# RiccZamboni/mepol

Hardware: AMD Instinct MI355X
Metric: MEPOL epoch wall-clock (C3: N=200000, d=29, k=30; rollout excluded) (lower is better)
Workload: dtype f64; 1 GPU; C3 Ant-shaped MEPOL epoch (k-NN + off-policy loop + final H); particles=200000, num_traj=400, traj_len=500, d=29, k=30, policy=29->[400, 300]->8 f64, parallelism=dp1

## Files before the change

### mepol_amd/csrc/wgrad.hip

```cpp
#include "mfma_f64.hpp"

#include <algorithm>

namespace mepol {
namespace wgrad {

using mfma::d4;
using mfma::frag_col;
using mfma::frag_row;
constexpr int FO = 4, FI = 5;
constexpr int kOcc = 2;
constexpr int BO = 16 * FO, BI = 16 * FI;
constexpr int NL = FO + FI;
constexpr int NS = 2;
constexpr bool kPin = true;
constexpr int kMaxSlices = 128;
constexpr int kSliceRowsMin = 256;

inline int slices_for(int64_t n, int O, int I) {
  const int64_t ntile = (int64_t)((O + BO - 1) / BO) * ((I + BI - 1) / BI);
  int64_t s = std::max<int64_t>(8, 1024 * kOcc / ntile);
  s = std::min<int64_t>(s, std::max<int64_t>(8, n / kSliceRowsMin));
  return (int)std::min<int64_t>(kMaxSlices, s & ~7);
}

inline size_t ws_bytes(int64_t n, int O, int I) {
  return (size_t)slices_for(n, O, I) * O * I * sizeof(double);
}

__global__ __launch_bounds__(64) __attribute__((amdgpu_waves_per_eu(kOcc))) void wgrad_kernel(
    const double* __restrict__ dy, int64_t n, int O, const double* __restrict__ x, int I,
    int nob, int nib, int S, int64_t slice_rows, double* __restrict__ part) {
  const int ntile = nob * nib;
  const int64_t b = blockIdx.x;
  const int64_t j = b >> 3;
  const int64_t s = (j / ntile) * 8 + (b & 7);
  const int tile = (int)(j % ntile);
  if (s >= S) return;
  const int ob = tile / nib, ib = tile % nib;
  const int l = threadIdx.x, fr = l & 15, g = l >> 4;
  const int64_t r_begin = s * slice_rows;
  const int64_t r_end = min(n, r_begin + slice_rows);
  if (r_begin >= r_end) {
    for (int t = 0; t < FO; ++t)
      for (int q = 0; q < 4; ++q) {
        const int o = ob * BO + 16 * t + frag_row(l, q);
        for (int u = 0; u < FI; ++u) {
          const int i = ib * BI + 16 * u + frag_col(l);
          if (o < O && i < I) part[((int64_t)s * O + o) * I + i] = 0.0;
        }
      }
    return;
  }
  int oc[FO], ic[FI];
#pragma unroll
  for (int t = 0; t < FO; ++t) oc[t] = min(ob * BO + 16 * t + fr, O - 1);
#pragma unroll
  for (int u = 0; u < FI; ++u) ic[u] = min(ib * BI + 16 * u + fr, I - 1);

  d4 acc[FO][FI];
#pragma unroll
  for (int t = 0; t < FO; ++t)
#pragma unroll
    for (int u = 0; u < FI; ++u) acc[t][u] = d4{0.0, 0.0, 0.0, 0.0};

  double R[NS][NL];
  auto load = [&](double (&D)[NL], int64_t ks) __attribute__((always_inline)) {
    const int64_t r = min(r_begin + 4 * ks + g, r_end - 1);
    const double* yr = dy + r * O;
    const double* xr = x + r * I;
#pragma unroll
    for (int t = 0; t < FO; ++t) D[t] = yr[oc[t]];
#pragma unroll
    for (int u = 0; u < FI; ++u) D[FO + u] = xr[ic[u]];
  };
  auto mma = [&](const double (&D)[NL]) __attribute__((always_inline)) {
#pragma unroll
    for (int t = 0; t < FO; ++t)
#pragma unroll
      for (int u = 0; u < FI; ++u)
        acc[t][u] = __builtin_amdgcn_mfma_f64_16x16x4f64(D[t], D[FO + u], acc[t][u], 0, 0, 0);
  };
  const int64_t rows = r_end - r_begin;
  const int64_t nfull = rows / 4;
  const int64_t nks = (rows + 3) / 4;
  mfma::ring_k_loop<NS, kPin>(
      nfull, nks, [&](int p, int64_t ks) __attribute__((always_inline)) { load(R[p], ks); },
      [&](int p, int64_t ks) __attribute__((always_inline)) {
        const bool ok = r_begin + 4 * ks + g < r_end;
#pragma unroll
        for (int v = 0; v < NL; ++v) R[p][v] = ok ? R[p][v] : 0.0;
      },
      [&](int p) __attribute__((always_inline)) { mma(R[p]); });
#pragma unroll
  for (int t = 0; t < FO; ++t)
#pragma unroll
    for (int q = 0; q < 4; ++q) {
      const int o = ob * BO + 16 * t + frag_row(l, q);
#pragma unroll
      for (int u = 0; u < FI; ++u) {
        const int i = ib * BI + 16 * u + frag_col(l);
        if (o < O && i < I) part[((int64_t)s * O + o) * I + i] = acc[t][u][q];
      }
    }
}

__global__ __launch_bounds__(256) void wgrad_reduce_kernel(const double* __restrict__ part, int S,
                                                          int64_t elems, double* __restrict__ out) {
  const int64_t e = (int64_t)blockIdx.x * 256 + threadIdx.x;
  if (e >= elems) return;
  double v = 0.0;
  for (int s = 0; s < S; s += 8) {
    double p[8];
#pragma unroll
    for (int u = 0; u < 8; ++u) p[u] = part[(int64_t)(s + u) * elems + e];
#pragma unroll
    for (int u = 0; u < 8; ++u) v += p[u];
  }
  out[e] = v;
}

}
}

extern "C" int mepol_weight_grad_workspace_size(int64_t n, int out_features, int in_features,
                                                size_t* bytes) {
  if (!bytes || n < 0 || out_features <= 0 || in_features <= 0) return mepol::kErrBadArg;
  *bytes = mepol::wgrad::ws_bytes(n, out_features, in_features);
  return 0;
}

extern "C" int mepol_weight_grad(const double* dy, int64_t n, int out_features, const double* x,
                                 int in_features, double* dW, void* workspace,
                                 size_t workspace_bytes, void* stream) {
  using namespace mepol::wgrad;
  const int O = out_features, I = in_features;
  if (n <= 0 || O <= 0 || I <= 0 || !dy || !x || !dW || !workspace) {
    mepol::set_error("mepol_weight_grad: bad arguments");
    return mepol::kErrBadArg;
  }
  const int S = slices_for(n, O, I);
  const size_t need = ws_bytes(n, O, I);
  if (workspace_bytes < need) {
    mepol::set_error("mepol_weight_grad: workspace %zu < %zu", workspace_bytes, need);
    return mepol::kErrWorkspace;
  }
  hipStream_t st = (hipStream_t)stream;
  const int nob = (O + BO - 1) / BO, nib = (I + BI - 1) / BI;
  const int64_t slice_rows = ((n + S - 1) / S + 3) / 4 * 4;
  const unsigned blocks = (unsigned)((int64_t)S * nob * nib);
  double* part = (double*)workspace;
  hipLaunchKernelGGL(wgrad_kernel, dim3(blocks), dim3(64), 0, st, dy, n, O, x, I, nob, nib, S,
                     slice_rows, part);
  MEPOL_CHECK_LAUNCH();
  const int64_t elems = (int64_t)O * I;
  hipLaunchKernelGGL(wgrad_reduce_kernel, dim3((unsigned)((elems + 255) / 256)), dim3(256), 0, st,
                     part, S, elems, dW);
  MEPOL_CHECK_LAUNCH();
  return 0;
}
```

Before: 0.1023 s/epoch.

## Split wgrad into full and short output tiles with XCD-aware slice scheduling

The weight-gradient kernel now handles the partial last output-row block separately, with a templated tile width (FOV) so short tiles issue fewer MFMAs and use a deeper pipeline. A host-side plan picks different split-K slice counts for full and short tiles and spreads blocks across the 8 XCDs with per-XCD capacity accounting. The reduce kernel is updated for the two partial layouts and non-multiple-of-8 slice counts. This aims to cut wasted MFMA work on padded rows and balance load across XCDs, at the cost of more complex scheduling logic and a kernel-wide branch.

```diff
diff --git a/mepol_amd/csrc/wgrad.hip b/mepol_amd/csrc/wgrad.hip
--- a/mepol_amd/csrc/wgrad.hip
+++ b/mepol_amd/csrc/wgrad.hip
@@ -11,75 +11,133 @@
 constexpr int FO = 4, FI = 5;
 constexpr int kOcc = 2;
 constexpr int BO = 16 * FO, BI = 16 * FI;
-constexpr int NL = FO + FI;
 constexpr int NS = 2;
+constexpr int kShortStages = 3;
 constexpr bool kPin = true;
 constexpr int kMaxSlices = 128;
 constexpr int kSliceRowsMin = 256;
 
-inline int slices_for(int64_t n, int O, int I) {
-  const int64_t ntile = (int64_t)((O + BO - 1) / BO) * ((I + BI - 1) / BI);
-  int64_t s = std::max<int64_t>(8, 1024 * kOcc / ntile);
-  s = std::min<int64_t>(s, std::max<int64_t>(8, n / kSliceRowsMin));
-  return (int)std::min<int64_t>(kMaxSlices, s & ~7);
+struct XcdMap {
+  int fend[8], send[8], fbase[8], sbase[8];
+};
+struct Plan {
+  int nob, nib, fol;
+  int Sf, Ss;
+  int64_t rows_f, rows_s;
+  int grid8;
+  XcdMap m;
+};
+constexpr int kXcdWaves = 1024 / 8 * kOcc;
+
+inline int64_t slice_rows_of(int64_t n, int S) { return ((n + S - 1) / S + 3) / 4 * 4; }
+
+inline Plan plan_for(int64_t n, int O, int I) {
+  Plan p{};
+  p.nob = (O + BO - 1) / BO;
+  p.nib = (I + BI - 1) / BI;
+  p.fol = (O - BO * (p.nob - 1) + 15) / 16;
+  const int nfo = p.nob - 1;
+  const int64_t lim = std::max<int64_t>(8, n / kSliceRowsMin);
+  const int64_t slots = 8 * kXcdWaves;
+  int64_t want_s;
+  if (nfo > 0) {
+    const int64_t sf = 4 * slots / ((int64_t)p.nib * (4 * nfo + p.fol));
+    p.Sf = (int)std::min<int64_t>({(int64_t)kMaxSlices, lim, std::max<int64_t>(8, sf)});
+    if ((int64_t)((p.Sf + 7) / 8) * nfo * p.nib > kXcdWaves) p.Sf = std::max(8, p.Sf & ~7);
+    want_s = ((int64_t)p.Sf * p.fol + 3) / 4;
+  } else {
+    want_s = slots / p.nib;
+  }
+  want_s = std::min<int64_t>({(int64_t)kMaxSlices, lim, std::max<int64_t>(8, want_s)});
+  const int tf = nfo * p.nib, ts = p.nib;
+  int nf[8], cap[8], ns[8];
+  int64_t capsum = 0;
+  for (int x = 0; x < 8; ++x) {
+    nf[x] = p.Sf / 8 + (x < p.Sf % 8 ? 1 : 0);
+    cap[x] = std::max(0, (kXcdWaves - nf[x] * tf) / ts);
+    capsum += cap[x];
+    ns[x] = 0;
+  }
+  if (capsum < 8)
+    for (int x = 0; x < 8; ++x) cap[x] = kMaxSlices;
+  else
+    want_s = std::min(want_s, capsum);
+  p.Ss = (int)want_s;
+  for (int left = p.Ss, x = 7; left > 0; x = (x + 7) % 8)
+    if (ns[x] < cap[x]) {
+      ++ns[x];
+      --left;
+    }
+  int fb = 0, sb = 0;
+  for (int x = 0; x < 8; ++x) {
+    p.m.fend[x] = nf[x] * tf;
+    p.m.send[x] = p.m.fend[x] + ns[x] * ts;
+    p.m.fbase[x] = fb;
+    p.m.sbase[x] = sb;
+    fb += nf[x];
+    sb += ns[x];
+    p.grid8 = std::max(p.grid8, p.m.send[x]);
+  }
+  p.rows_f = p.Sf ? slice_rows_of(n, p.Sf) : 0;
+  p.rows_s = slice_rows_of(n, p.Ss);
+  return p;
 }
 
 inline size_t ws_bytes(int64_t n, int O, int I) {
-  return (size_t)slices_for(n, O, I) * O * I * sizeof(double);
-}
-
-__global__ __launch_bounds__(64) __attribute__((amdgpu_waves_per_eu(kOcc))) void wgrad_kernel(
-    const double* __restrict__ dy, int64_t n, int O, const double* __restrict__ x, int I,
-    int nob, int nib, int S, int64_t slice_rows, double* __restrict__ part) {
-  const int ntile = nob * nib;
-  const int64_t b = blockIdx.x;
-  const int64_t j = b >> 3;
-  const int64_t s = (j / ntile) * 8 + (b & 7);
-  const int tile = (int)(j % ntile);
-  if (s >= S) return;
-  const int ob = tile / nib, ib = tile % nib;
+  const Plan p = plan_for(n, O, I);
+  const int64_t of = (int64_t)BO * (p.nob - 1);
+  return (size_t)(p.Sf * of + p.Ss * (O - of)) * I * sizeof(double);
+}
+
+template <int FOV>
+__device__ __forceinline__ void wgrad_tile(const double* __restrict__ dy, int64_t n, int O,
+                                           const double* __restrict__ x, int I, int o0, int g0,
+                                           int og, int ib, int64_t s, int64_t slice_rows,
+                                           double* __restrict__ part) {
+  constexpr int NLV = FOV + FI;
+  constexpr int NS = FOV < FO ? kShortStages : wgrad::NS;
   const int l = threadIdx.x, fr = l & 15, g = l >> 4;
   const int64_t r_begin = s * slice_rows;
   const int64_t r_end = min(n, r_begin + slice_rows);
   if (r_begin >= r_end) {
-    for (int t = 0; t < FO; ++t)
+    for (int t = 0; t < FOV; ++t)
       for (int q = 0; q < 4; ++q) {
-        const int o = ob * BO + 16 * t + frag_row(l, q);
+        const int o = o0 + 16 * t + frag_row(l, q);
         for (int u = 0; u < FI; ++u) {
           const int i = ib * BI + 16 * u + frag_col(l);
-          if (o < O && i < I) part[((int64_t)s * O + o) * I + i] = 0.0;
+          if (o < O && i < I) part[((int64_t)s * og + o - g0) * I + i] = 0.0;
         }
       }
     return;
   }
-  int oc[FO], ic[FI];
-#pragma unroll
-  for (int t = 0; t < FO; ++t) oc[t] = min(ob * BO + 16 * t + fr, O - 1);
+  int oc[FOV], ic[FI];
+#pragma unroll
+  for (int t = 0; t < FOV; ++t) oc[t] = min(o0 + 16 * t + fr, O - 1);
 #pragma unroll
   for (int u = 0; u < FI; ++u) ic[u] = min(ib * BI + 16 * u + fr, I - 1);
 
-  d4 acc[FO][FI];
-#pragma unroll
-  for (int t = 0; t < FO; ++t)
+  d4 acc[FOV][FI];
+#pragma unroll
+  for (int t = 0; t < FOV; ++t)
 #pragma unroll
     for (int u = 0; u < FI; ++u) acc[t][u] = d4{0.0, 0.0, 0.0, 0.0};
 
-  double R[NS][NL];
-  auto load = [&](double (&D)[NL], int64_t ks) __attribute__((always_inline)) {
+  double R[NS][NLV];
+  auto load = [&](double (&D)[NLV], int64_t ks) __attribute__((always_inline)) {
     const int64_t r = min(r_begin + 4 * ks + g, r_end - 1);
     const double* yr = dy + r * O;
     const double* xr = x + r * I;
 #pragma unroll
-    for (int t = 0; t < FO; ++t) D[t] = yr[oc[t]];
-#pragma unroll
-    for (int u = 0; u < FI; ++u) D[FO + u] = xr[ic[u]];
+    for (int t = 0; t < FOV; ++t) D[t] = yr[oc[t]];
+#pragma unroll
+    for (int u = 0; u < FI; ++u) D[FOV + u] = xr[ic[u]];
   };
-  auto mma = [&](const double (&D)[NL]) __attribute__((always_inline)) {
-#pragma unroll
-    for (int t = 0; t < FO; ++t)
+  auto mma = [&](const double (&D)[NLV]) __attribute__((always_inline)) {
+#pragma unroll
+    for (int t = 0; t < FOV; ++t)
 #pragma unroll
       for (int u = 0; u < FI; ++u)
-        acc[t][u] = __builtin_amdgcn_mfma_f64_16x16x4f64(D[t], D[FO + u], acc[t][u], 0, 0, 0);
+        acc[t][u] = __builtin_amdgcn_mfma_f64_16x16x4f64(D[t], D[FOV + u], acc[t][u], 0, 0, 0);
   };
   const int64_t rows = r_end - r_begin;
   const int64_t nfull = rows / 4;
@@ -89,33 +147,70 @@
       [&](int p, int64_t ks) __attribute__((always_inline)) {
         const bool ok = r_begin + 4 * ks + g < r_end;
 #pragma unroll
-        for (int v = 0; v < NL; ++v) R[p][v] = ok ? R[p][v] : 0.0;
+        for (int v = 0; v < NLV; ++v) R[p][v] = ok ? R[p][v] : 0.0;
       },
       [&](int p) __attribute__((always_inline)) { mma(R[p]); });
 #pragma unroll
-  for (int t = 0; t < FO; ++t)
+  for (int t = 0; t < FOV; ++t)
 #pragma unroll
     for (int q = 0; q < 4; ++q) {
-      const int o = ob * BO + 16 * t + frag_row(l, q);
+      const int o = o0 + 16 * t + frag_row(l, q);
 #pragma unroll
       for (int u = 0; u < FI; ++u) {
         const int i = ib * BI + 16 * u + frag_col(l);
-        if (o < O && i < I) part[((int64_t)s * O + o) * I + i] = acc[t][u][q];
+        if (o < O && i < I) part[((int64_t)s * og + o - g0) * I + i] = acc[t][u][q];
       }
     }
 }
 
-__global__ __launch_bounds__(256) void wgrad_reduce_kernel(const double* __restrict__ part, int S,
-                                                          int64_t elems, double* __restrict__ out) {
+__global__ __launch_bounds__(64) __attribute__((amdgpu_waves_per_eu(kOcc))) void wgrad_kernel(
+    const double* __restrict__ dy, int64_t n, int O, const double* __restrict__ x, int I,
+    int nob, int nib, int fol, int Sf, int64_t rows_f, int64_t rows_s, XcdMap m,
+    double* __restrict__ part) {
+  const int xcd = blockIdx.x & 7;
+  int j = blockIdx.x >> 3;
+  const int of = BO * (nob - 1);
+  int fo, o0, g0, og, ib;
+  int64_t s, rows;
+  if (j < m.fend[xcd]) {
+    const int tf = (nob - 1) * nib, tile = j % tf;
+    fo = FO, o0 = (tile / nib) * BO, g0 = 0, og = of, ib = tile % nib;
+    s = m.fbase[xcd] + j / tf, rows = rows_f;
+  } else if (j < m.send[xcd]) {
+    j -= m.fend[xcd];
+    fo = fol, o0 = of, g0 = of, og = O - of, ib = j % nib;
+    s = m.sbase[xcd] + j / nib, rows = rows_s;
+    part += (int64_t)Sf * of * I;
+  } else {
+    return;
+  }
+  if (fo == 4)
+    wgrad_tile<4>(dy, n, O, x, I, o0, g0, og, ib, s, rows, part);
+  else if (fo == 3)
+    wgrad_tile<3>(dy, n, O, x, I, o0, g0, og, ib, s, rows, part);
+  else if (fo == 2)
+    wgrad_tile<2>(dy, n, O, x, I, o0, g0, og, ib, s, rows, part);
+  else
+    wgrad_tile<1>(dy, n, O, x, I, o0, g0, og, ib, s, rows, part);
+}
+
+__global__ __launch_bounds__(256) void wgrad_reduce_kernel(const double* __restrict__ part, int of,
+                                                          int Sf, int Ss, int O, int I,
+                                                          double* __restrict__ out) {
   const int64_t e = (int64_t)blockIdx.x * 256 + threadIdx.x;
-  if (e >= elems) return;
+  if (e >= (int64_t)O * I) return;
+  const bool full = e < (int64_t)of * I;
+  const int S = full ? Sf : Ss;
+  const int64_t stride = (int64_t)(full ? of : O - of) * I;
+  const double* p0 = full ? part + e : part + (int64_t)Sf * of * I + (e - (int64_t)of * I);
   double v = 0.0;
   for (int s = 0; s < S; s += 8) {
     double p[8];
 #pragma unroll
-    for (int u = 0; u < 8; ++u) p[u] = part[(int64_t)(s + u) * elems + e];
-#pragma unroll
-    for (int u = 0; u < 8; ++u) v += p[u];
+    for (int u = 0; u < 8; ++u) p[u] = p0[min(s + u, S - 1) * stride];
+#pragma unroll
+    for (int u = 0; u < 8; ++u)
+      v = s + u < S ? v + p[u] : v;
   }
   out[e] = v;
 }
@@ -139,23 +234,21 @@
     mepol::set_error("mepol_weight_grad: bad arguments");
     return mepol::kErrBadArg;
   }
-  const int S = slices_for(n, O, I);
+  const Plan p = plan_for(n, O, I);
   const size_t need = ws_bytes(n, O, I);
   if (workspace_bytes < need) {
     mepol::set_error("mepol_weight_grad: workspace %zu < %zu", workspace_bytes, need);
     return mepol::kErrWorkspace;
   }
   hipStream_t st = (hipStream_t)stream;
-  const int nob = (O + BO - 1) / BO, nib = (I + BI - 1) / BI;
-  const int64_t slice_rows = ((n + S - 1) / S + 3) / 4 * 4;
-  const unsigned blocks = (unsigned)((int64_t)S * nob * nib);
+  const unsigned blocks = 8u * (unsigned)p.grid8;
   double* part = (double*)workspace;
-  hipLaunchKernelGGL(wgrad_kernel, dim3(blocks), dim3(64), 0, st, dy, n, O, x, I, nob, nib, S,
-                     slice_rows, part);
+  hipLaunchKernelGGL(wgrad_kernel, dim3(blocks), dim3(64), 0, st, dy, n, O, x, I, p.nob, p.nib,
+                     p.fol, p.Sf, p.rows_f, p.rows_s, p.m, part);
   MEPOL_CHECK_LAUNCH();
   const int64_t elems = (int64_t)O * I;
   hipLaunchKernelGGL(wgrad_reduce_kernel, dim3((unsigned)((elems + 255) / 256)), dim3(256), 0, st,
-                     part, S, elems, dW);
+                     part, BO * (p.nob - 1), p.Sf, p.Ss, O, I, dW);
   MEPOL_CHECK_LAUNCH();
   return 0;
 }
```

After: 0.1011 s/epoch, median of 6. 1.1% less time.
